# kishwarshafin/pepper

Hardware: AMD Instinct MI355X
Metric: inference windows/sec (whole node) (higher is better)
Workload: dtype f32 via f16 hi/lo split operands (3 MFMAs per product), f32 accumulate

## Files before the change

pepper_amd/build.py:

```python
import os
import shutil
import subprocess
import sys

CSRC = os.path.join(os.path.dirname(os.path.abspath(__file__)), "csrc")
LIB = os.path.join(CSRC, "libpepper_amd.so")
SOURCES = ["api.hip", "inflate.hip", "gemm.hip", "gemm_h2.hip", "rnn.hip", "rnn_h2.hip", "mlp_h2.hip", "head.hip", "encoder.hip", "encoder_polish.hip", "realign.hip"]
HEADERS = ["common.h", "kernels.h", "encoder_common.h", "reservoir.h", "candidates.h", "pack_rule.h", "dec_frag16.h", os.path.join("..", "..", "include", "pepper_amd.h"),
           os.path.join("..", "..", "include", "pepper_amd_encoder.h"),
           os.path.join("..", "..", "include", "pepper_amd_realign.h")]


def _hipcc():
    for cand in (os.environ.get("HIPCC"), shutil.which("hipcc"), "/opt/rocm/bin/hipcc"):
        if cand and os.path.exists(cand):
            return cand
    raise RuntimeError("hipcc not found (set HIPCC)")


IO_LIB = os.path.join(CSRC, "libpepper_amd_io.so")
HDF5_PREFIX = os.environ.get("PEPPER_AMD_HDF5_PREFIX", "/opt/conda")


def _have_libdeflate(inc, lib):
    if os.environ.get("PEPPER_AMD_LIBDEFLATE", "1") == "0":
        return False
    return os.path.exists(os.path.join(inc, "libdeflate.h")) and os.path.exists(os.path.join(lib, "libdeflate.so"))


def build_io(force=False, verbose=False):
    src = os.path.join(CSRC, "hdf5io.cpp")
    bam = os.path.join(CSRC, "bamio.cpp")
    bld = os.path.join(CSRC, "h5build.cpp")
    cnd = os.path.join(CSRC, "candidates.cpp")
    hdr = os.path.join(CSRC, "..", "..", "include", "pepper_amd_io.h")
    rsv = os.path.join(CSRC, "reservoir.h")
    pkr = os.path.join(CSRC, "pack_rule.h")
    have_src = all(os.path.exists(f) for f in (src, bam, bld, cnd, hdr, rsv, pkr))
    if os.path.exists(IO_LIB) and (not have_src or (not force and os.path.getmtime(IO_LIB) >= max(
            os.path.getmtime(src), os.path.getmtime(bam), os.path.getmtime(bld), os.path.getmtime(cnd), os.path.getmtime(hdr),
            os.path.getmtime(rsv), os.path.getmtime(pkr)))):
        return IO_LIB
    inc, lib = os.path.join(HDF5_PREFIX, "include"), os.path.join(HDF5_PREFIX, "lib")
    if not os.path.exists(os.path.join(inc, "hdf5.h")):
        raise RuntimeError(f"hdf5.h not found under {inc}: set PEPPER_AMD_HDF5_PREFIX")
    tmp = f"{IO_LIB}.{os.getpid()}.tmp"
    cmd = ["g++", "-O2", "-std=c++17", "-shared", "-fPIC", "-o", tmp, src, bam, bld, cnd, f"-I{inc}",
           os.path.join(lib, "libhdf5.so"), "-lz", "-lpthread", f"-Wl,-rpath,{lib}", "-Wl,--no-undefined"]
    if _have_libdeflate(inc, lib):
        cmd += ["-DPA_HAVE_LIBDEFLATE=1", os.path.join(lib, "libdeflate.so")]
    if verbose:
        print(" ".join(cmd), file=sys.stderr)
    try:
        subprocess.run(cmd, check=True)
        os.replace(tmp, IO_LIB)
    finally:
        if os.path.exists(tmp):
            os.remove(tmp)
    return IO_LIB


TOOLS = os.path.join(os.path.dirname(os.path.dirname(os.path.abspath(__file__))), "tools")
SYNTH_BAM = os.path.join(TOOLS, "synth_bam")


def build_tools(force=False):
    src = os.path.join(TOOLS, "synth_bam.cpp")
    if not os.path.exists(src):
        return SYNTH_BAM if os.path.exists(SYNTH_BAM) else None
    if not force and os.path.exists(SYNTH_BAM) and os.path.getmtime(SYNTH_BAM) >= os.path.getmtime(src):
        return SYNTH_BAM
    inc, lib = os.path.join(HDF5_PREFIX, "include"), os.path.join(HDF5_PREFIX, "lib")
    tmp = f"{SYNTH_BAM}.{os.getpid()}.tmp"
    cmd = ["g++", "-O2", "-std=c++17", "-o", tmp, src, "-lz", "-lpthread"]
    if _have_libdeflate(inc, lib):
        cmd += [f"-I{inc}", "-DPA_HAVE_LIBDEFLATE=1", os.path.join(lib, "libdeflate.so"), f"-Wl,-rpath,{lib}"]
    try:
        subprocess.run(cmd, check=True)
        os.replace(tmp, SYNTH_BAM)
    finally:
        if os.path.exists(tmp):
            os.remove(tmp)
    return SYNTH_BAM


OBJ_DIR = os.path.join(CSRC, "_obj")


def _flags():
    return ["--offload-arch=gfx950", "-O3", "-std=c++17", "-fPIC", "-Xarch_host", "-mf16c", "-Wno-unused-result"] + \
        os.environ.get("PEPPER_AMD_EXTRA_HIPCC_FLAGS", "").split()


def _same_flags():
    stamp = os.path.join(OBJ_DIR, "flags.txt")
    return not os.path.exists(stamp) or open(stamp).read() == " ".join(_flags())


def needs_build():
    if not os.path.exists(LIB):
        return True
    t = os.path.getmtime(LIB)
    return not _same_flags() or any(os.path.getmtime(os.path.join(CSRC, f)) > t for f in SOURCES + HEADERS)


def build(force=False, verbose=False):
    if not force and not needs_build():
        return LIB
    flags = _flags()
    os.makedirs(OBJ_DIR, exist_ok=True)
    stamp = os.path.join(OBJ_DIR, "flags.txt")
    same_flags = os.path.exists(stamp) and open(stamp).read() == " ".join(flags)
    newest_header = max(os.path.getmtime(os.path.join(CSRC, h)) for h in HEADERS)
    todo = []
    for src in SOURCES:
        obj = os.path.join(OBJ_DIR, src + ".o")
        if force or not same_flags or not os.path.exists(obj) or os.path.getmtime(obj) < max(
                newest_header, os.path.getmtime(os.path.join(CSRC, src))):
            todo.append((src, obj))

    def compile_one(item):
        src, obj = item
        cmd = [_hipcc()] + flags + ["-c", src, "-o", obj + f".{os.getpid()}.tmp"]
        if verbose:
            print(" ".join(cmd), file=sys.stderr)
        subprocess.run(cmd, cwd=CSRC, check=True)
        os.replace(obj + f".{os.getpid()}.tmp", obj)
    if todo:
        from concurrent.futures import ThreadPoolExecutor
        with ThreadPoolExecutor(max_workers=min(len(todo), os.cpu_count() or 4)) as pool:
            list(pool.map(compile_one, todo))
    with open(stamp, "w") as fh:
        fh.write(" ".join(flags))
    tmp = f"{LIB}.{os.getpid()}.tmp"
    cmd = [_hipcc(), "--offload-arch=gfx950", "-shared", "-fPIC", "-o", tmp] + [os.path.join(OBJ_DIR, s + ".o") for s in SOURCES]
    if verbose:
        print(" ".join(cmd), file=sys.stderr)
    try:
        subprocess.run(cmd, cwd=CSRC, check=True)
        os.replace(tmp, LIB)
    finally:
        if os.path.exists(tmp):
            os.remove(tmp)
    return LIB


if __name__ == "__main__":
    print(build(force=True, verbose=True))
    print(build_io(force=True, verbose=True))
    print(build_tools(force=True))
```

pepper_amd/csrc/rnn_h2.hip:

```cpp
#include <cstdlib>

#include "common.h"
#include "kernels.h"

namespace {

typedef _Float16 h8 __attribute__((ext_vector_type(8)));

constexpr int MT = 64;

PA_DEV f32x16 mfma_h(h8 a, h8 b, f32x16 c) { return __builtin_amdgcn_mfma_f32_32x32x16_f16(a, b, c, 0, 0, 0); }

PA_DEV void decode_block(int bid, int& dir, int& btile) {
    const int xcd = bid & 7, q = bid >> 3;
    dir = xcd >> 2;
    btile = q * 4 + (xcd & 3);
}



template <int MTILES>
PA_DEV void lstm_dec_h2_body(const float* __restrict__ bias, const uint32_t* __restrict__ Wp, uint32_t* __restrict__ Y, int ldy,
                             int B, int T, unsigned long long* __restrict__ dbg, const uint32_t* __restrict__ Xh, int ldxh);
template <int MTILES, bool BC>
PA_DEV void lstm_enc_h2_body(const int8_t* __restrict__ Xi, int F, const float* __restrict__ bias, const uint32_t* __restrict__ Wp,
                             uint32_t* __restrict__ Y, int ldy, int B, int T, unsigned long long* __restrict__ dbg);

template <int H, int KX, bool XG = false, int SAUX = 0, bool BC = false, int MTILES = 2>
__global__ __launch_bounds__(H / 32 * 64, 1) void lstm_rec_h2_kernel(const float* __restrict__ Xp, int ldx,
                                                                     const int8_t* __restrict__ Xi, int F,
                                                                     const float* __restrict__ bias,
                                                                     const uint32_t* __restrict__ Wp,
                                                                     uint32_t* __restrict__ Y, int ldy, int B, int T,
                                                                     unsigned long long* __restrict__ dbg,
                                                                     const uint32_t* __restrict__ Xh = nullptr, int ldxh = 0) {
    if constexpr (XG) {
        static_assert(H == 256 && KX == 512 && SAUX == 2 && !BC, "the fused decoder has one shape");
        lstm_dec_h2_body<MTILES>(bias, Wp, Y, ldy, B, T, dbg, Xh, ldxh);
        return;
    }
    if constexpr (!XG && KX == 32) {
        static_assert(H == 256 && SAUX == 2, "the fused int8 encoder has one shape");
        lstm_enc_h2_body<MTILES, BC>(Xi, F, bias, Wp, Y, ldy, B, T, dbg);
        return;
    }
    constexpr int KT = H + KX, KS = KT / 16, KSH = H / 16, NT = H / 32, NW = H / 32;
    constexpr int MTL = 32 * MTILES;
    static_assert(MTILES == 1 || MTILES == 2, "32 or 64 rows per workgroup");
    constexpr int ROWB = KT * 4 + 16;
    constexpr int ROWD = ROWB / 4;
    extern __shared__ __attribute__((aligned(16))) uint32_t lds[];
    static_assert(KS % 2 == 0, "the weight prefetch assumes an even number of k steps");
    static_assert((ROWB / 16) % 2 == 1, "row stride must be an odd number of 16-byte slots");

    int dir, btile;
    decode_block(blockIdx.x, dir, btile);
    const int b0 = btile * MTL;
    if (b0 >= B) return;

    const int tid = threadIdx.x, lane = tid & 63;
    const int u = __builtin_amdgcn_readfirstlane(tid >> 6);
    const int li = lane & 31, hf = lane >> 5;

    float* cs = reinterpret_cast<float*>(lds + MTL * ROWD) + u * (MTILES * 16 * 64) + lane;
    for (int idx = tid; idx < MTL * ROWD + NW * MTILES * 16 * 64; idx += blockDim.x) lds[idx] = 0u;

    f32x16 acc[MTILES][4];

    const size_t urow = (size_t)b0 * T;
    const __amdgpu_buffer_rsrc_t xrs = __builtin_amdgcn_make_buffer_rsrc(
        const_cast<float*>(KX ? bias + dir * 4 * H + 32 * u : Xp + (size_t)(b0 >> 5) * T * (ldx >> 5) * 1024), 0,
        0x7fffffff, 0x00020000);
    const __amdgpu_buffer_rsrc_t wrs = __builtin_amdgcn_make_buffer_rsrc(
        const_cast<uint32_t*>(Wp + ((size_t)dir * (4 * NT) + u) * KS * 512), 0, 0x7fffffff, 0x00020000);
    const unsigned xoff = KX ? li * 4u : lane * 16u;
    const unsigned woff = lane * 16u;

    auto seed_chunk = [&](int m, int qd, int t) {
        if (KX) return;
#pragma unroll
        for (int g = 0; g < 4; ++g) {
            {
                const unsigned ct = (unsigned)(dir * (4 * NT) + g * NT + u);
                const unsigned so = (((unsigned)(m * T + t) * (ldx >> 5) + ct) * 4u + qd) * 1024u;
                const f32x4 v = __builtin_bit_cast(f32x4, __builtin_amdgcn_raw_buffer_load_b128(xrs, xoff, so, 0));
                acc[m][g][4 * qd] = v.x;
                acc[m][g][4 * qd + 1] = v.y;
                acc[m][g][4 * qd + 2] = v.z;
                acc[m][g][4 * qd + 3] = v.w;
            }
        }
    };

    constexpr bool XI8 = KX > 0;
    constexpr int XN = XI8 ? (MTL * KX / 2) / (NW * 64) : 1;
    unsigned xv[XN];
    auto x_load = [&](int t) {
        if (XI8) {
#pragma unroll
            for (int k = 0; k < XN; ++k) {
                const int e = tid + k * (NW * 64);
                const int row = e / (KX / 2), f = (e % (KX / 2)) * 2;
                int brow = b0 + row;
                brow = brow < B ? brow : B - 1;
                const int8_t* src = Xi + ((size_t)brow * T + t) * F;
                const _Float16 one = BC ? (_Float16)1.0f : (_Float16)0.0f;
                const _Float16 h0 = f < F ? (_Float16)(float)src[f] : (f == F ? one : (_Float16)0.0f);
                const _Float16 h1 = f + 1 < F ? (_Float16)(float)src[f + 1] : (f + 1 == F ? one : (_Float16)0.0f);
                xv[k] = (unsigned)__builtin_bit_cast(unsigned short, h0) |
                        ((unsigned)__builtin_bit_cast(unsigned short, h1) << 16);
            }
        }
    };
    auto x_store = [&]() {
        if (XI8) {
#pragma unroll
            for (int k = 0; k < XN; ++k) {
                const int e = tid + k * (NW * 64);
                const int row = e / (KX / 2), f = (e % (KX / 2)) * 2;
                lds[row * ROWD + ((H + f) >> 3) * 8 + ((f & 7) >> 1)] = xv[k];
            }
        }
    };
    struct Frag { h8 b[4][2], a[MTILES][2]; };
    const uint32_t* arow = lds + li * ROWD + hf * 8;
    auto load_b = [&](int s, Frag& fr) {
#pragma unroll
        for (int g = 0; g < 4; ++g)
#pragma unroll
            for (int hl = 0; hl < 2; ++hl)
                fr.b[g][hl] = __builtin_bit_cast(h8, __builtin_amdgcn_raw_buffer_load_b128(
                                                         wrs, woff, (unsigned)((g * NT * KS + s) * 2 + hl) * 1024u, 0));
    };
    auto load_a = [&](int s, Frag& fr, int) {
#pragma unroll
        for (int m = 0; m < MTILES; ++m) {
            fr.a[m][0] = *reinterpret_cast<const h8*>(arow + m * 32 * ROWD + s * 16);
            fr.a[m][1] = *reinterpret_cast<const h8*>(arow + m * 32 * ROWD + s * 16 + 4);
        }
    };

    constexpr int CPR = H / 4;
    constexpr int YROWS = (NW * 64) / CPR;
    constexpr int YC = MTL / YROWS;
    const int yc_row = tid / CPR, yc_c = tid % CPR;
    const uint32_t* yc_src = lds + yc_row * ROWD + yc_c * 4;
    const __amdgpu_buffer_rsrc_t ycrs =
        __builtin_amdgcn_make_buffer_rsrc(Y + urow * ldy + dir * H, 0, 0x7fffffff, 0x00020000);
    const unsigned yc_off = ((unsigned)(yc_row * T) * ldy + yc_c * 4) * 4u;
    auto yc_read = [&](int j) { return *reinterpret_cast<const u32x4*>(yc_src + j * YROWS * ROWD); };
    auto yc_write = [&](int j, int tp, u32x4 v) {
        __builtin_amdgcn_raw_buffer_store_b128(v, ycrs, yc_off, ((unsigned)(j * YROWS * T + tp) * ldy) * 4u, SAUX);
    };

    const int hcol = 32 * u + li;
    unsigned short* hl_dst = reinterpret_cast<unsigned short*>(lds + 4 * hf * ROWD + (hcol >> 3) * 8 + ((hcol & 7) >> 1)) + (hcol & 1);
    const bool odd = li & 1;

    Frag ring[2];
    __syncthreads();
    {
        const int t0 = dir ? T - 1 : 0;
#pragma unroll
        for (int m = 0; m < MTILES; ++m)
#pragma unroll
            for (int qd = 0; qd < 4; ++qd) seed_chunk(m, qd, t0);
        x_load(t0);
        x_store();
        load_b(0, ring[0]);
    }
    __syncthreads();

    for (int step = 0; step < T; ++step) {
        const int t = dir ? T - 1 - step : step;
        const bool stamp = dbg != nullptr && blockIdx.x == 8 && lane == 0;
        if (stamp) dbg[(u * 80 + 2 * step) * 2] = __builtin_amdgcn_s_memtime();
        {
            load_a(0, ring[0], t);
            const int tp = step > 0 ? (dir ? t + 1 : t - 1) : t;
            u32x4 ycv = {0, 0, 0, 0};
#pragma unroll
            for (int s = 0; s < KS; ++s) {
                const int p = s & 1;
                if (s + 1 < KS) { load_b(s + 1, ring[p ^ 1]); load_a(s + 1, ring[p ^ 1], t); }
                else load_b(0, ring[p ^ 1]);
                if (s >= 1 && s <= YC) yc_write(s - 1, tp, ycv);
                if (s < YC) ycv = yc_read(s);
#pragma unroll
                for (int term = 0; term < 3; ++term) {
                    if (XI8 && s >= KSH && term == 0) continue;
                    const bool fresh = KX && s == 0 && term == 0;
#pragma unroll
                    for (int g = 0; g < 4; ++g)
#pragma unroll
                        for (int m = 0; m < MTILES; ++m)
                            acc[m][g] = mfma_h(ring[p].a[m][term == 0 ? 1 : 0], ring[p].b[g][term == 1 ? 1 : 0],
                                               fresh ? f32x16{} : acc[m][g]);
                }
                if (MTILES == 1 && s + 1 < KS) {
#pragma unroll
                    for (int q = 0; q < 8; ++q) {
                        __builtin_amdgcn_sched_group_barrier(0x008, 1, 0);
                        __builtin_amdgcn_sched_group_barrier(0x020, 1, 0);
                    }
#pragma unroll
                    for (int q = 0; q < 2; ++q) {
                        __builtin_amdgcn_sched_group_barrier(0x008, 1, 0);
                        __builtin_amdgcn_sched_group_barrier(0x100, 1, 0);
                    }
                    if (s <= YC) {
                        __builtin_amdgcn_sched_group_barrier(0x008, 1, 0);
                        __builtin_amdgcn_sched_group_barrier(0x040, 1, 0);
                        __builtin_amdgcn_sched_group_barrier(0x008, 1, 0);
                        __builtin_amdgcn_sched_group_barrier(0x100, 1, 0);
                    } else {
                        __builtin_amdgcn_sched_group_barrier(0x008, 2, 0);
                    }
                } else if (s + 1 < KS) {
#pragma unroll
                    for (int q = 0; q < 8; ++q) {
                        __builtin_amdgcn_sched_group_barrier(0x008, 2, 0);
                        __builtin_amdgcn_sched_group_barrier(0x020, 1, 0);
                    }
#pragma unroll
                    for (int q = 0; q < 4; ++q) {
                        __builtin_amdgcn_sched_group_barrier(0x008, 1, 0);
                        __builtin_amdgcn_sched_group_barrier(0x100, 1, 0);
                    }
                    if (s <= YC) {
                        __builtin_amdgcn_sched_group_barrier(0x008, 1, 0);
                        __builtin_amdgcn_sched_group_barrier(0x040, 1, 0);
                        __builtin_amdgcn_sched_group_barrier(0x008, 1, 0);
                        __builtin_amdgcn_sched_group_barrier(0x100, 1, 0);
                        __builtin_amdgcn_sched_group_barrier(0x008, 2, 0);
                    } else {
                        __builtin_amdgcn_sched_group_barrier(0x008, 4, 0);
                    }
                } else if (MTILES == 1) {
#pragma unroll
                    for (int q = 0; q < 8; ++q) {
                        __builtin_amdgcn_sched_group_barrier(0x008, 1, 0);
                        __builtin_amdgcn_sched_group_barrier(0x020, 1, 0);
                    }
                    __builtin_amdgcn_sched_group_barrier(0x008, 4, 0);
                } else {
#pragma unroll
                    for (int q = 0; q < 8; ++q) {
                        __builtin_amdgcn_sched_group_barrier(0x008, 2, 0);
                        __builtin_amdgcn_sched_group_barrier(0x020, 1, 0);
                    }
                    __builtin_amdgcn_sched_group_barrier(0x008, 8, 0);
                }
                __builtin_amdgcn_sched_barrier(0);
            }
        }
        float cb[4] = {0.0f, 0.0f, 0.0f, 0.0f};
        if (KX && !BC) {
#pragma unroll
            for (int g = 0; g < 4; ++g)
                cb[g] = __builtin_bit_cast(float, __builtin_amdgcn_raw_buffer_load_b32(xrs, xoff, (unsigned)(g * H) * 4u, 0));
        }
        if (stamp) dbg[(u * 80 + 2 * step) * 2 + 1] = __builtin_amdgcn_s_memtime();

        lds_barrier();
        if (stamp) dbg[(u * 80 + 2 * step + 1) * 2] = __builtin_amdgcn_s_memtime();

        const int tn = dir ? t - 1 : t + 1;
        if (step + 1 < T) x_load(tn);
#pragma unroll
        for (int m = 0; m < MTILES; ++m)
#pragma unroll
            for (int qd = 0; qd < 4; ++qd) {
#pragma unroll
                for (int e = 0; e < 4; e += 2) {
                    const int r = 4 * qd + e;
                    typedef float f32x2 __attribute__((ext_vector_type(2)));
                    const f32x2 one = {1.0f, 1.0f};
                    f32x2 ai = {acc[m][0][r], acc[m][0][r + 1]}, af = {acc[m][1][r], acc[m][1][r + 1]},
                          ag = {acc[m][2][r], acc[m][2][r + 1]}, ao = {acc[m][3][r], acc[m][3][r + 1]};
                    if (KX && !BC) { ai += cb[0]; af += cb[1]; ag += cb[2]; ao += cb[3]; }
                    auto ex2 = [](f32x2 v) { return f32x2{__builtin_amdgcn_exp2f(v.x), __builtin_amdgcn_exp2f(v.y)}; };
                    auto rcp = [](f32x2 v) { return f32x2{__builtin_amdgcn_rcpf(v.x), __builtin_amdgcn_rcpf(v.y)}; };
                    const f32x2 ig = rcp(one + ex2(ai));
                    const f32x2 fg = rcp(one + ex2(af));
                    const f32x2 gg = one - 2.0f * rcp(one + ex2(ag));
                    const f32x2 og = rcp(one + ex2(ao));
                    const f32x2 cold = {cs[(m * 16 + r) * 64], cs[(m * 16 + r + 1) * 64]};
                    const f32x2 cn = fg * cold + ig * gg;
                    cs[(m * 16 + r) * 64] = cn.x;
                    cs[(m * 16 + r + 1) * 64] = cn.y;
                    const f32x2 hv2 = og * (one - 2.0f * rcp(one + ex2(cn * 2.8853900817779268f)));
#pragma unroll
                    for (int k = 0; k < 2; ++k) {
                        const float hv = k ? hv2.y : hv2.x;
                        h2_store16(hl_dst + (32 * m + ((r + k) & 3) + 8 * ((r + k) >> 2)) * ROWD * 2, hv);
                    }
                }
                if (step + 1 < T) seed_chunk(m, qd, tn);
            }
        if (step + 1 < T) x_store();
        if (stamp) dbg[(u * 80 + 2 * step + 1) * 2 + 1] = __builtin_amdgcn_s_memtime();
        lds_barrier();
    }
    {
        const int tl = dir ? 0 : T - 1;
#pragma unroll
        for (int j = 0; j < YC; ++j) yc_write(j, tl, yc_read(j));
    }
}

template <bool FRESH_, bool Y_, bool Y2_, int XR_, int AN_>
struct DecStep {
    static constexpr bool FRESH = FRESH_, Y = Y_, Y2 = Y2_;
    static constexpr int XR = XR_, AN = AN_;
};

template <int MTILES>
PA_DEV void lstm_dec_h2_body(const float* __restrict__ bias, const uint32_t* __restrict__ Wp, uint32_t* __restrict__ Y, int ldy,
                             int B, int T, unsigned long long* __restrict__ dbg, const uint32_t* __restrict__ Xh, int ldxh) {
    constexpr int H = 256, KX = 512, KS = (H + KX) / 32, KSH = H / 32, NW = H / 32, SAUX = 2;
    constexpr int MTL = 32 * MTILES, RT = 2 * MTILES;
    static_assert(MTILES == 1 || MTILES == 2, "32 or 64 rows per workgroup");
    constexpr int ROWB = H * 4 + 16, ROWD = ROWB / 4;
    extern __shared__ __attribute__((aligned(16))) uint32_t lds[];
    static_assert((ROWB / 16) % 2 == 1, "row stride must be an odd number of 16-byte slots");

    int dir, btile;
    decode_block(blockIdx.x, dir, btile);
    const int b0 = btile * MTL;
    if (b0 >= B) return;

    const int tid = threadIdx.x, lane = tid & 63;
    const int u = __builtin_amdgcn_readfirstlane(tid >> 6);
    const int lr = lane & 15, lq = lane >> 4;

    float* cs = reinterpret_cast<float*>(lds + MTL * ROWD) + u * (MTILES * 16 * 64) + lane;
    for (int idx = tid; idx < MTL * ROWD + NW * MTILES * 16 * 64; idx += blockDim.x) lds[idx] = 0u;
    constexpr int XRD = 36, XSLOT = MTL * XRD;
    uint32_t* xring = lds + MTL * ROWD + NW * MTILES * 16 * 64;

    f32x4 acc[RT][4][2];

    const size_t urow = (size_t)b0 * T;
    const __amdgpu_buffer_rsrc_t brs =
        __builtin_amdgcn_make_buffer_rsrc(const_cast<float*>(bias + dir * 4 * H + 32 * u), 0, 0x7fffffff, 0x00020000);
    const __amdgpu_buffer_rsrc_t wrs = __builtin_amdgcn_make_buffer_rsrc(
        const_cast<uint32_t*>(Wp + ((size_t)dir * (4 * 16) + 2 * u) * KS * 512), 0, 0x7fffffff, 0x00020000);
    const unsigned woff = lane * 16u;

    const bool xg_stager = tid < MTL * 8;
    const __amdgpu_buffer_rsrc_t xgrs =
        __builtin_amdgcn_make_buffer_rsrc(const_cast<uint32_t*>(Xh + (size_t)b0 * T * ldxh), 0, 0x7fffffff, 0x00020000);
    const unsigned xg_off = ((unsigned)((tid >> 3) * T) * ldxh) * 4u + (tid & 7) * 16u;
    uint32_t* xst_dst = xring + (tid >> 3) * XRD + (tid & 7) * 4;
    u32x4 xstage = {0, 0, 0, 0};
    auto xg_load = [&](int j, int t) {
        if (MTILES == 2 || xg_stager)
            xstage = __builtin_amdgcn_raw_buffer_load_b128(xgrs, xg_off, ((unsigned)t * ldxh) * 4u + (unsigned)j * 128u, SAUX);
    };
    auto xg_store = [&](int slot) {
        if (MTILES == 2 || xg_stager) *reinterpret_cast<u32x4*>(xst_dst + slot * XSLOT) = xstage;
    };

    int once = 1;
    asm volatile("" : "+s"(once));
    h8 a[RT][2];
    h8 b[2][2][2][2];
    const uint32_t* arow = lds + lr * ROWD + lq * 8;
    const uint32_t* xrow = xring + lr * XRD + lq * 8;
    auto load_b = [&](int s, int gp, int idx) {
        const int c = idx >> 2, hl = (idx >> 1) & 1, g2 = idx & 1;
        b[gp][g2][c][hl] = __builtin_bit_cast(
            h8, __builtin_amdgcn_raw_buffer_load_b128(wrs, woff, (unsigned)((((2 * gp + g2) * 16 + c) * KS + s) * 2 + hl) * 1024u, 0));
    };
    auto load_a_h = [&](int s, int m, int hl) { a[m][hl] = *reinterpret_cast<const h8*>(arow + m * 16 * ROWD + s * 32 + hl * 4); };
    auto load_a_x = [&](int slot, int m, int hl) {
        a[m][hl] = *reinterpret_cast<const h8*>(xrow + slot * XSLOT + m * 16 * XRD + hl * 4);
    };

    constexpr int CPR = H / 4;
    constexpr int YROWS = (NW * 64) / CPR;
    constexpr int YC = MTL / YROWS;
    const int yc_row = tid / CPR, yc_c = tid % CPR;
    const uint32_t* yc_src = lds + yc_row * ROWD + yc_c * 4;
    const __amdgpu_buffer_rsrc_t ycrs =
        __builtin_amdgcn_make_buffer_rsrc(Y + urow * ldy + dir * H, 0, 0x7fffffff, 0x00020000);
    const unsigned yc_off = ((unsigned)(yc_row * T) * ldy + yc_c * 4) * 4u;
    auto yc_read = [&](int j) { return *reinterpret_cast<const u32x4*>(yc_src + j * YROWS * ROWD); };
    auto yc_write = [&](int j, int tp, u32x4 v) {
        __builtin_amdgcn_raw_buffer_store_b128(v, ycrs, yc_off, ((unsigned)(j * YROWS * T + tp) * ldy) * 4u, SAUX);
    };

    const int hcol = 32 * u + lr;
    unsigned short* hl_dst = reinterpret_cast<unsigned short*>(lds + 4 * lq * ROWD + (hcol >> 3) * 8 + ((hcol & 7) >> 1)) + (hcol & 1);

    __syncthreads();
#pragma unroll
    for (int i = 0; i < 8; ++i) load_b(0, 0, i);
    __syncthreads();

    for (int step = 0; step < T; ++step) {
        const int t = dir ? T - 1 - step : step;
        const bool stamp = dbg != nullptr && blockIdx.x == 8 && lane == 0;
        if (stamp) dbg[(u * 80 + 2 * step) * 2] = __builtin_amdgcn_s_memtime();
        {
            const int tp = step > 0 ? (dir ? t + 1 : t - 1) : t;
            u32x4 ycv = {0, 0, 0, 0}, ycv2 = {0, 0, 0, 0};
            constexpr int NM = RT * 12;
            auto kstep = [&](int s, auto cfg) {
                using C = decltype(cfg);
                const int sn = C::AN == 0 ? 0 : s + 1, slot = (s - KSH + 1) & 1;
#pragma unroll
                for (int gp = 0; gp < 2; ++gp) {
                    if (gp == 1 && C::XR == 2) lds_barrier();
#pragma unroll
                    for (int i = 0; i < NM; ++i) {
                        const int m = i / 12, c = (i % 12) / 6, term = (i % 6) >> 1, g2 = i & 1, g = 2 * gp + g2;
                        acc[m][g][c] = __builtin_amdgcn_mfma_f32_16x16x32_f16(a[m][term == 0 ? 1 : 0], b[gp][g2][c][term == 1 ? 1 : 0],
                                                                              C::FRESH && term == 0 ? f32x4{} : acc[m][g][c], 0, 0, 0);
                        if (MTILES == 2 ? (i < 24 && i % 3 == 1) : i < 8) load_b(gp == 0 ? s : sn, gp ^ 1, MTILES == 2 ? i / 3 : i);
                        if (gp == 1 && C::AN != 0 && (i % 12 == 9 || i % 12 == 11)) {
                            if (C::AN == 1) load_a_h(sn, m, i % 12 == 9 ? 1 : 0);
                            else load_a_x(slot, m, i % 12 == 9 ? 1 : 0);
                        }
                        if (C::Y && i == NM / 2 + 1) {
                            if (gp == 0) ycv = yc_read(s);
                            else yc_write(s, tp, ycv);
                        }
                        if (C::Y2 && i == NM / 2 + 4) {
                            if (gp == 0) ycv2 = yc_read(YC - 1);
                            else yc_write(YC - 1, tp, ycv2);
                        }
                        if (C::XR == 2 && gp == 0 && i == NM - 1) xg_store(slot);
                        if (C::XR != 0 && gp == 1 && i == (MTILES == 2 ? 2 : 10)) xg_load(s - 6 < KS - KSH ? s - 6 : KS - KSH - 1, t);
                        __builtin_amdgcn_sched_barrier(0);
                    }
                }
            };
            constexpr bool Y2 = YC > 7;
            constexpr int YL = YC < 6 ? YC : 6;
#pragma unroll
            for (int i = 0; i < 2 * RT; ++i) load_a_h(0, i >> 1, i & 1);
            __builtin_amdgcn_sched_barrier(0);
#pragma unroll 1
            for (int r = 0; r < once; ++r) kstep(0, DecStep<true, true, Y2, 0, 1>{});
#pragma unroll 1
            for (int s = 1; s < YL; ++s) kstep(s, DecStep<false, true, false, 0, 1>{});
#pragma unroll 1
            for (int s = YL; s < 6; ++s) kstep(s, DecStep<false, false, false, 0, 1>{});
#pragma unroll 1
            for (int r = 0; r < once; ++r) kstep(6, DecStep<false, (YC > 6), false, 1, 1>{});
#pragma unroll 1
            for (int s = 7; s < KS - 1; ++s) kstep(s, DecStep<false, false, false, 2, 2>{});
#pragma unroll 1
            for (int r = 0; r < once; ++r) kstep(KS - 1, DecStep<false, false, false, 0, 0>{});
        }
        float cb[4][2];
#pragma unroll
        for (int g = 0; g < 4; ++g)
#pragma unroll
            for (int c = 0; c < 2; ++c)
                cb[g][c] = __builtin_bit_cast(float, __builtin_amdgcn_raw_buffer_load_b32(brs, lr * 4u, (unsigned)(g * H + 16 * c) * 4u, 0));
        if (stamp) dbg[(u * 80 + 2 * step) * 2 + 1] = __builtin_amdgcn_s_memtime();

        lds_barrier();
        if (stamp) dbg[(u * 80 + 2 * step + 1) * 2] = __builtin_amdgcn_s_memtime();

#pragma unroll
        for (int m = 0; m < RT; ++m)
#pragma unroll
            for (int c = 0; c < 2; ++c)
#pragma unroll
                for (int e = 0; e < 4; e += 2) {
                    typedef float f32x2 __attribute__((ext_vector_type(2)));
                    const f32x2 one = {1.0f, 1.0f};
                    f32x2 ai = {acc[m][0][c][e], acc[m][0][c][e + 1]}, af = {acc[m][1][c][e], acc[m][1][c][e + 1]},
                          ag = {acc[m][2][c][e], acc[m][2][c][e + 1]}, ao = {acc[m][3][c][e], acc[m][3][c][e + 1]};
                    ai += cb[0][c]; af += cb[1][c]; ag += cb[2][c]; ao += cb[3][c];
                    auto ex2 = [](f32x2 v) { return f32x2{__builtin_amdgcn_exp2f(v.x), __builtin_amdgcn_exp2f(v.y)}; };
                    auto rcp = [](f32x2 v) { return f32x2{__builtin_amdgcn_rcpf(v.x), __builtin_amdgcn_rcpf(v.y)}; };
                    const f32x2 ig = rcp(one + ex2(ai));
                    const f32x2 fg = rcp(one + ex2(af));
                    const f32x2 gg = one - 2.0f * rcp(one + ex2(ag));
                    const f32x2 og = rcp(one + ex2(ao));
                    const int ci = (m * 8 + c * 4 + e) * 64;
                    const f32x2 cold = {cs[ci], cs[ci + 64]};
                    const f32x2 cn = fg * cold + ig * gg;
                    cs[ci] = cn.x;
                    cs[ci + 64] = cn.y;
                    const f32x2 hv2 = og * (one - 2.0f * rcp(one + ex2(cn * 2.8853900817779268f)));
#pragma unroll
                    for (int k = 0; k < 2; ++k) h2_store16(hl_dst + (16 * m + e + k) * ROWD * 2 + c * 32, k ? hv2.y : hv2.x);
                }
        if (stamp) dbg[(u * 80 + 2 * step + 1) * 2 + 1] = __builtin_amdgcn_s_memtime();
        lds_barrier();
    }
    {
        const int tl = dir ? 0 : T - 1;
#pragma unroll
        for (int j = 0; j < YC; ++j) yc_write(j, tl, yc_read(j));
    }
}

#ifndef PA_ENC_SKIP0
#define PA_ENC_SKIP0 1
#endif
template <bool FRESH_, bool Y_, bool X_, int AN_>
struct EncStep {
    static constexpr bool FRESH = FRESH_, Y = Y_, X = X_;
    static constexpr int AN = AN_;
};

template <int MTILES, bool BC>
PA_DEV void lstm_enc_h2_body(const int8_t* __restrict__ Xi, int F, const float* __restrict__ bias, const uint32_t* __restrict__ Wp,
                             uint32_t* __restrict__ Y, int ldy, int B, int T, unsigned long long* __restrict__ dbg) {
    constexpr int H = 256, KX = 32, KS = (H + KX) / 32, KSH = H / 32, NW = H / 32, SAUX = 2;
    constexpr int MTL = 32 * MTILES, RT = 2 * MTILES;
    static_assert(MTILES == 1 || MTILES == 2, "32 or 64 rows per workgroup");
    constexpr int ROWB = (H + KX) * 4 + 16, ROWD = ROWB / 4;
    extern __shared__ __attribute__((aligned(16))) uint32_t lds[];
    static_assert((ROWB / 16) % 2 == 1, "row stride must be an odd number of 16-byte slots");

    int dir, btile;
    decode_block(blockIdx.x, dir, btile);
    const int b0 = btile * MTL;
    if (b0 >= B) return;

    const int tid = threadIdx.x, lane = tid & 63;
    const int u = __builtin_amdgcn_readfirstlane(tid >> 6);
    const int lr = lane & 15, lq = lane >> 4;

    float* cs = reinterpret_cast<float*>(lds + MTL * ROWD) + u * (MTILES * 16 * 64) + lane;
    for (int idx = tid; idx < MTL * ROWD + NW * MTILES * 16 * 64; idx += blockDim.x) lds[idx] = 0u;

    f32x4 acc[RT][4][2];

    const size_t urow = (size_t)b0 * T;
    const __amdgpu_buffer_rsrc_t brs =
        __builtin_amdgcn_make_buffer_rsrc(const_cast<float*>(bias + dir * 4 * H + 32 * u), 0, 0x7fffffff, 0x00020000);
    const __amdgpu_buffer_rsrc_t wrs = __builtin_amdgcn_make_buffer_rsrc(
        const_cast<uint32_t*>(Wp + ((size_t)dir * (4 * 16) + 2 * u) * KS * 512), 0, 0x7fffffff, 0x00020000);
    const unsigned woff = lane * 16u;

    constexpr int XN = (MTL * KX / 2) / (NW * 64);
    unsigned xv[XN];
    auto x_load = [&](int t) {
#pragma unroll
        for (int k = 0; k < XN; ++k) {
            const int e = tid + k * (NW * 64);
            const int row = e / (KX / 2), f = (e % (KX / 2)) * 2;
            int brow = b0 + row;
            brow = brow < B ? brow : B - 1;
            const int8_t* src = Xi + ((size_t)brow * T + t) * F;
            const _Float16 one = BC ? (_Float16)1.0f : (_Float16)0.0f;
            const _Float16 h0 = f < F ? (_Float16)(float)src[f] : (f == F ? one : (_Float16)0.0f);
            const _Float16 h1 = f + 1 < F ? (_Float16)(float)src[f + 1] : (f + 1 == F ? one : (_Float16)0.0f);
            xv[k] = (unsigned)__builtin_bit_cast(unsigned short, h0) | ((unsigned)__builtin_bit_cast(unsigned short, h1) << 16);
        }
    };
    auto x_store = [&]() {
#pragma unroll
        for (int k = 0; k < XN; ++k) {
            const int e = tid + k * (NW * 64);
            const int row = e / (KX / 2), f = (e % (KX / 2)) * 2;
            lds[row * ROWD + ((H + f) >> 3) * 8 + ((f & 7) >> 1)] = xv[k];
        }
    };

    int once = 1;
    asm volatile("" : "+s"(once));
    h8 a[RT][2];
    h8 b[2][2][2][2];
    const uint32_t* arow = lds + lr * ROWD + lq * 8;
    auto load_b = [&](int s, int gp, int idx) {
        const int c = idx >> 2, hl = (idx >> 1) & 1, g2 = idx & 1;
        b[gp][g2][c][hl] = __builtin_bit_cast(
            h8, __builtin_amdgcn_raw_buffer_load_b128(wrs, woff, (unsigned)((((2 * gp + g2) * 16 + c) * KS + s) * 2 + hl) * 1024u, 0));
    };
    auto load_a = [&](int s, int m, int hl) { a[m][hl] = *reinterpret_cast<const h8*>(arow + m * 16 * ROWD + s * 32 + hl * 4); };

    constexpr int CPR = H / 4;
    constexpr int YROWS = (NW * 64) / CPR;
    constexpr int YC = MTL / YROWS;
    static_assert(YC <= KSH, "one y copy pass per h k step");
    const int yc_row = tid / CPR, yc_c = tid % CPR;
    const uint32_t* yc_src = lds + yc_row * ROWD + yc_c * 4;
    const __amdgpu_buffer_rsrc_t ycrs =
        __builtin_amdgcn_make_buffer_rsrc(Y + urow * ldy + dir * H, 0, 0x7fffffff, 0x00020000);
    const unsigned yc_off = ((unsigned)(yc_row * T) * ldy + yc_c * 4) * 4u;
    auto yc_read = [&](int j) { return *reinterpret_cast<const u32x4*>(yc_src + j * YROWS * ROWD); };
    auto yc_write = [&](int j, int tp, u32x4 v) {
        __builtin_amdgcn_raw_buffer_store_b128(v, ycrs, yc_off, ((unsigned)(j * YROWS * T + tp) * ldy) * 4u, SAUX);
    };

    const int hcol = 32 * u + lr;
    unsigned short* hl_dst = reinterpret_cast<unsigned short*>(lds + 4 * lq * ROWD + (hcol >> 3) * 8 + ((hcol & 7) >> 1)) + (hcol & 1);

    __syncthreads();
    {
        x_load(dir ? T - 1 : 0);
        x_store();
#pragma unroll
        for (int i = 0; i < 8; ++i) load_b(PA_ENC_SKIP0 ? KS - 1 : 0, 0, i);
    }
    __syncthreads();

    for (int step = 0; step < T; ++step) {
        const int t = dir ? T - 1 - step : step;
        const bool stamp = dbg != nullptr && blockIdx.x == 8 && lane == 0;
        if (stamp) dbg[(u * 80 + 2 * step) * 2] = __builtin_amdgcn_s_memtime();
        {
            const int tp = step > 0 ? (dir ? t + 1 : t - 1) : t;
            u32x4 ycv = {0, 0, 0, 0};
            auto kstep = [&](int s, auto cfg) {
                using C = decltype(cfg);
                constexpr int PT = C::X ? 4 : 6;
                constexpr int NM = RT * 2 * PT;
                const int sn = C::X ? 0 : s + 1;
#pragma unroll
                for (int gp = 0; gp < 2; ++gp) {
#pragma unroll
                    for (int i = 0; i < NM; ++i) {
                        const int m = i / (2 * PT), c = (i % (2 * PT)) / PT, term = ((i % PT) >> 1) + (C::X ? 1 : 0), g2 = i & 1,
                                  g = 2 * gp + g2;
                        acc[m][g][c] = __builtin_amdgcn_mfma_f32_16x16x32_f16(a[m][term == 0 ? 1 : 0], b[gp][g2][c][term == 1 ? 1 : 0],
                                                                              C::FRESH && i % PT < 2 ? f32x4{} : acc[m][g][c], 0, 0, 0);
                        if (C::X) {
                            if (MTILES == 2 ? (i < 16 && (i & 1)) : i < 8) load_b(gp == 0 ? s : sn, gp ^ 1, MTILES == 2 ? i >> 1 : i);
                        } else {
                            if (MTILES == 2 ? (i < 24 && i % 3 == 1) : i < 8) load_b(gp == 0 ? s : sn, gp ^ 1, MTILES == 2 ? i / 3 : i);
                        }
                        if (!C::X && gp == 1 && C::AN == 1 && i % 12 == 9) load_a(sn, m, 1);
                        if (!C::X && gp == 1 && C::AN != 0 && i % 12 == 11) load_a(sn, m, 0);
                        if (C::Y && i == NM / 2 + 1) {
                            if (gp == 0) ycv = yc_read(s);
                            else yc_write(s, tp, ycv);
                        }
                        __builtin_amdgcn_sched_barrier(0);
                    }
                }
            };
            const int hrun = PA_ENC_SKIP0 && step == 0 ? 0 : once;
#pragma unroll
            for (int i = 0; i < 2 * RT; ++i) load_a(0, i >> 1, i & 1);
            __builtin_amdgcn_sched_barrier(0);
#pragma unroll 1
            for (int r = 0; r < hrun; ++r) kstep(0, EncStep<true, true, false, 1>{});
#pragma unroll 1
            for (int s = 1; s < (YC < KSH - 1 ? YC : KSH - 1) * hrun; ++s) kstep(s, EncStep<false, true, false, 1>{});
            if constexpr (YC < KSH - 1) {
#pragma unroll 1
                for (int s = YC; s < (KSH - 1) * hrun; ++s) kstep(s, EncStep<false, false, false, 1>{});
            }
#pragma unroll 1
            for (int r = 0; r < hrun; ++r) kstep(KSH - 1, EncStep<false, (YC >= KSH), false, 2>{});
#pragma unroll 1
            for (int r = 0; r < hrun; ++r) kstep(KS - 1, EncStep<false, false, true, 0>{});
            if (PA_ENC_SKIP0) {
#pragma unroll 1
                for (int r = hrun; r < once; ++r) {
#pragma unroll
                    for (int m = 0; m < RT; ++m) load_a(KSH, m, 0);
                    __builtin_amdgcn_sched_barrier(0);
                    kstep(KS - 1, EncStep<true, false, true, 0>{});
                }
            }
        }
        float cb[4][2] = {};
        if (!BC) {
#pragma unroll
            for (int g = 0; g < 4; ++g)
#pragma unroll
                for (int c = 0; c < 2; ++c)
                    cb[g][c] = __builtin_bit_cast(float, __builtin_amdgcn_raw_buffer_load_b32(brs, lr * 4u, (unsigned)(g * H + 16 * c) * 4u, 0));
        }
        if (stamp) dbg[(u * 80 + 2 * step) * 2 + 1] = __builtin_amdgcn_s_memtime();

        lds_barrier();
        if (stamp) dbg[(u * 80 + 2 * step + 1) * 2] = __builtin_amdgcn_s_memtime();

        const int tn = dir ? t - 1 : t + 1;
        if (step + 1 < T) x_load(tn);
#pragma unroll
        for (int m = 0; m < RT; ++m)
#pragma unroll
            for (int c = 0; c < 2; ++c)
#pragma unroll
                for (int e = 0; e < 4; e += 2) {
                    typedef float f32x2 __attribute__((ext_vector_type(2)));
                    const f32x2 one = {1.0f, 1.0f};
                    f32x2 ai = {acc[m][0][c][e], acc[m][0][c][e + 1]}, af = {acc[m][1][c][e], acc[m][1][c][e + 1]},
                          ag = {acc[m][2][c][e], acc[m][2][c][e + 1]}, ao = {acc[m][3][c][e], acc[m][3][c][e + 1]};
                    if (!BC) { ai += cb[0][c]; af += cb[1][c]; ag += cb[2][c]; ao += cb[3][c]; }
                    auto ex2 = [](f32x2 v) { return f32x2{__builtin_amdgcn_exp2f(v.x), __builtin_amdgcn_exp2f(v.y)}; };
                    auto rcp = [](f32x2 v) { return f32x2{__builtin_amdgcn_rcpf(v.x), __builtin_amdgcn_rcpf(v.y)}; };
                    const f32x2 ig = rcp(one + ex2(ai));
                    const f32x2 fg = rcp(one + ex2(af));
                    const f32x2 gg = one - 2.0f * rcp(one + ex2(ag));
                    const f32x2 og = rcp(one + ex2(ao));
                    const int ci = (m * 8 + c * 4 + e) * 64;
                    const f32x2 cold = {cs[ci], cs[ci + 64]};
                    const f32x2 cn = fg * cold + ig * gg;
                    cs[ci] = cn.x;
                    cs[ci + 64] = cn.y;
                    const f32x2 hv2 = og * (one - 2.0f * rcp(one + ex2(cn * 2.8853900817779268f)));
#pragma unroll
                    for (int k = 0; k < 2; ++k) h2_store16(hl_dst + (16 * m + e + k) * ROWD * 2 + c * 32, k ? hv2.y : hv2.x);
                }
        if (step + 1 < T) x_store();
        if (stamp) dbg[(u * 80 + 2 * step + 1) * 2 + 1] = __builtin_amdgcn_s_memtime();
        lds_barrier();
    }
    {
        const int tl = dir ? 0 : T - 1;
#pragma unroll
        for (int j = 0; j < YC; ++j) yc_write(j, tl, yc_read(j));
    }
}

constexpr int US_AUX_SC1 = 16;

template <int H, int NTW>
__global__ __launch_bounds__(256, 1) void lstm_rec_h2_split_kernel(const float* __restrict__ Xp, int ldx,
                                                                   const uint32_t* __restrict__ Wp, uint32_t* __restrict__ Y,
                                                                   int ldy, int B, int T, uint32_t* __restrict__ exch,
                                                                   unsigned* __restrict__ counters, int* __restrict__ failed,
                                                                   int tiles4, int sabotage) {
    static_assert(H == 256 && (NTW == 1 || NTW == 2), "eight members of 32 units or four of 64");
    constexpr int KS = H / 16, NT = H / 32, K = NT / NTW;
    constexpr int ROWB = H * 4 + 16, ROWD = ROWB / 4;
    extern __shared__ __attribute__((aligned(16))) uint32_t lds[];
    float* gbuf = reinterpret_cast<float*>(lds + 32 * ROWD);
    uint32_t* flag = lds + 32 * ROWD + 4 * NTW * 16 * 64;

    const int xcd = blockIdx.x & 7, q = blockIdx.x >> 3;
    const int dir = xcd >> 2, member = q % K, btile = (q / K) * 4 + (xcd & 3);
    const int b0 = btile * 32;
    if (b0 >= B) return;
    const int group = dir * tiles4 + btile;

    const int tid = threadIdx.x, lane = tid & 63;
    const int w = __builtin_amdgcn_readfirstlane(tid >> 6);
    const int li = lane & 31, hf = lane >> 5;
    for (int idx = tid; idx < 32 * ROWD; idx += 256) lds[idx] = 0u;
    if (tid == 0) *flag = 0u;

    h8 bw[NTW][KS][2];
    {
        const __amdgpu_buffer_rsrc_t wrs = __builtin_amdgcn_make_buffer_rsrc(
            const_cast<uint32_t*>(Wp + (size_t)dir * (4 * NT) * KS * 512), 0, 0x7fffffff, 0x00020000);
#pragma unroll
        for (int j = 0; j < NTW; ++j)
#pragma unroll
            for (int s = 0; s < KS; ++s)
#pragma unroll
                for (int hl = 0; hl < 2; ++hl)
                    bw[j][s][hl] = __builtin_bit_cast(h8, __builtin_amdgcn_raw_buffer_load_b128(
                                                              wrs, lane * 16u,
                                                              (unsigned)(((w * NT + member * NTW + j) * KS + s) * 2 + hl) * 1024u, 0));
    }
    const __amdgpu_buffer_rsrc_t xrs = __builtin_amdgcn_make_buffer_rsrc(
        const_cast<float*>(Xp + (size_t)btile * T * (ldx >> 5) * 1024), 0, 0x7fffffff, 0x00020000);
    const unsigned ct0 = (unsigned)(dir * (4 * NT) + w * NT + member * NTW);
    f32x16 acc[NTW];
    auto seed = [&](int t) {
#pragma unroll
        for (int j = 0; j < NTW; ++j)
#pragma unroll
            for (int qd = 0; qd < 4; ++qd) {
                const unsigned so = (((unsigned)t * (ldx >> 5) + ct0 + j) * 4u + qd) * 1024u;
                const f32x4 v = __builtin_bit_cast(f32x4, __builtin_amdgcn_raw_buffer_load_b128(xrs, lane * 16u, so, 0));
                acc[j][4 * qd] = v.x;
                acc[j][4 * qd + 1] = v.y;
                acc[j][4 * qd + 2] = v.z;
                acc[j][4 * qd + 3] = v.w;
            }
    };

    const uint32_t* arow = lds + li * ROWD + hf * 8;
    const int hcol = 32 * member * NTW + li;
    unsigned short* hl_dst = reinterpret_cast<unsigned short*>(lds + 4 * hf * ROWD + (hcol >> 3) * 8 + ((hcol & 7) >> 1)) + (hcol & 1);
    const int xrow = tid >> 3, xc = tid & 7;
    const __amdgpu_buffer_rsrc_t ers = __builtin_amdgcn_make_buffer_rsrc(
        exch + (size_t)group * 2 * 32 * H, 0, 0x7fffffff, 0x00020000);
    const __amdgpu_buffer_rsrc_t yrs = __builtin_amdgcn_make_buffer_rsrc(
        Y + (size_t)b0 * T * ldy + dir * H, 0, 0x7fffffff, 0x00020000);
    unsigned* cnt = counters + group * 32;

    float c[NTW][4];
#pragma unroll
    for (int j = 0; j < NTW; ++j)
#pragma unroll
        for (int e = 0; e < 4; ++e) c[j][e] = 0.0f;
    seed(dir ? T - 1 : 0);
    __syncthreads();

    for (int step = 0; step < T; ++step) {
        const int t = dir ? T - 1 - step : step;
        {
            h8 a0 = *reinterpret_cast<const h8*>(arow), a1 = *reinterpret_cast<const h8*>(arow + 4);
#pragma unroll
            for (int s = 0; s < KS; ++s) {
                h8 n0 = a0, n1 = a1;
                if (s + 1 < KS) {
                    n0 = *reinterpret_cast<const h8*>(arow + (s + 1) * 16);
                    n1 = *reinterpret_cast<const h8*>(arow + (s + 1) * 16 + 4);
                }
#pragma unroll
                for (int j = 0; j < NTW; ++j) acc[j] = mfma_h(a1, bw[j][s][0], acc[j]);
#pragma unroll
                for (int j = 0; j < NTW; ++j) acc[j] = mfma_h(a0, bw[j][s][1], acc[j]);
#pragma unroll
                for (int j = 0; j < NTW; ++j) acc[j] = mfma_h(a0, bw[j][s][0], acc[j]);
                a0 = n0;
                a1 = n1;
            }
        }
#pragma unroll
        for (int j = 0; j < NTW; ++j)
#pragma unroll
            for (int r = 0; r < 16; ++r) {
                const float sg = __builtin_amdgcn_rcpf(1.0f + __builtin_amdgcn_exp2f(acc[j][r]));
                gbuf[((w * NTW + j) * 16 + r) * 64 + lane] = w == 2 ? 1.0f - 2.0f * sg : sg;
            }
        if (step + 1 < T) seed(dir ? t - 1 : t + 1);
        lds_barrier();
#pragma unroll
        for (int j = 0; j < NTW; ++j)
#pragma unroll
            for (int e = 0; e < 4; ++e) {
                const int r = 4 * w + e;
                const float ig = gbuf[((0 * NTW + j) * 16 + r) * 64 + lane], fg = gbuf[((1 * NTW + j) * 16 + r) * 64 + lane];
                const float gg = gbuf[((2 * NTW + j) * 16 + r) * 64 + lane], og = gbuf[((3 * NTW + j) * 16 + r) * 64 + lane];
                const float cn = fg * c[j][e] + ig * gg;
                c[j][e] = cn;
                const float hv = og * (1.0f - 2.0f * __builtin_amdgcn_rcpf(1.0f + __builtin_amdgcn_exp2f(cn * 2.8853900817779268f)));
                h2_store16(hl_dst + j * 64 + (e + 8 * w) * ROWD * 2, hv);
            }
        lds_barrier();
        const unsigned pbase = (unsigned)(step & 1) * (32u * H * 4u);
#pragma unroll
        for (int j = 0; j < NTW; ++j) {
            const int chunk = (member * NTW + j) * 8 + xc;
            const u32x4 mine = *reinterpret_cast<const u32x4*>(lds + xrow * ROWD + chunk * 4);
            __builtin_amdgcn_raw_buffer_store_b128(mine, yrs, ((unsigned)(xrow * T) * ldy + chunk * 4) * 4u, ((unsigned)t * ldy) * 4u, 0);
            if (step + 1 < T)
                __builtin_amdgcn_raw_buffer_store_b128(mine, ers, (unsigned)(xrow * H + chunk * 4) * 4u, pbase, US_AUX_SC1);
        }
        if (step + 1 == T) break;
        __builtin_amdgcn_s_waitcnt(0);
        __builtin_amdgcn_s_barrier();
        if (tid == 0) {
            if (!(sabotage && group == 0 && member == K - 1))
                __hip_atomic_fetch_add(cnt, 1u, __ATOMIC_RELAXED, __HIP_MEMORY_SCOPE_AGENT);
            const unsigned want = (unsigned)K * (unsigned)(step + 1);
            const int bound = step == 0 ? (1 << 13) : (1 << 11);
            int spins = 0;
            while (__hip_atomic_load(cnt, __ATOMIC_RELAXED, __HIP_MEMORY_SCOPE_AGENT) < want) {
// ... 870 lines not shown
```

Baseline: 2.732 million.

## Fold LSTM gate math into fewer transcendentals and skip zero-state decoder step

Moves the LSTM cell nonlinearity into a shared header and adds a form that merges the input and candidate gates, and the output gate with the tanh of the cell, into single reciprocals, with clamped exponent arguments. The aim is to cut exp/rcp instructions in the serial recurrent step. The decoder also gains a step-zero path that skips the recurrent h-matmul k-steps, since the initial hidden state is zero, and loads the x operand earlier. The new gate form changes rounding slightly, and the step-zero path adds control-flow complexity to the k-step schedule.

After: 2.731 million (median of 2 runs). No clear change (-0.0%).

```diff
diff --git a/pepper_amd/build.py b/pepper_amd/build.py
--- a/pepper_amd/build.py
+++ b/pepper_amd/build.py
@@ -6,7 +6,7 @@
 CSRC = os.path.join(os.path.dirname(os.path.abspath(__file__)), "csrc")
 LIB = os.path.join(CSRC, "libpepper_amd.so")
 SOURCES = ["api.hip", "inflate.hip", "gemm.hip", "gemm_h2.hip", "rnn.hip", "rnn_h2.hip", "mlp_h2.hip", "head.hip", "encoder.hip", "encoder_polish.hip", "realign.hip"]
-HEADERS = ["common.h", "kernels.h", "encoder_common.h", "reservoir.h", "candidates.h", "pack_rule.h", "dec_frag16.h", os.path.join("..", "..", "include", "pepper_amd.h"),
+HEADERS = ["common.h", "kernels.h", "encoder_common.h", "reservoir.h", "candidates.h", "pack_rule.h", "dec_frag16.h", "lstm_gate.h", os.path.join("..", "..", "include", "pepper_amd.h"),
            os.path.join("..", "..", "include", "pepper_amd_encoder.h"),
            os.path.join("..", "..", "include", "pepper_amd_realign.h")]
 
diff --git a/pepper_amd/csrc/lstm_gate.h b/pepper_amd/csrc/lstm_gate.h
--- /dev/null
+++ b/pepper_amd/csrc/lstm_gate.h
@@ -0,0 +1,64 @@
+#pragma once
+#include <math.h>
+
+#ifndef PA_LSTM_GATE_FORM
+#define PA_LSTM_GATE_FORM 8
+#endif
+#if PA_LSTM_GATE_FORM != 10 && PA_LSTM_GATE_FORM != 8
+#error "PA_LSTM_GATE_FORM is 10 or 8"
+#endif
+
+namespace pa_gate {
+
+#if defined(__HIPCC__)
+#define PA_GATE_FN __host__ __device__ __forceinline__
+#else
+#define PA_GATE_FN inline
+#endif
+#if defined(__clang__)
+typedef float f32x2 __attribute__((ext_vector_type(2)));
+#else
+struct f32x2 {
+    float x, y;
+};
+inline f32x2 operator+(f32x2 a, f32x2 b) { return f32x2{a.x + b.x, a.y + b.y}; }
+inline f32x2 operator-(f32x2 a, f32x2 b) { return f32x2{a.x - b.x, a.y - b.y}; }
+inline f32x2 operator*(f32x2 a, f32x2 b) { return f32x2{a.x * b.x, a.y * b.y}; }
+#endif
+#if defined(__HIP_DEVICE_COMPILE__)
+PA_GATE_FN f32x2 ex2(f32x2 v) { return f32x2{__builtin_amdgcn_exp2f(v.x), __builtin_amdgcn_exp2f(v.y)}; }
+PA_GATE_FN f32x2 rcp(f32x2 v) { return f32x2{__builtin_amdgcn_rcpf(v.x), __builtin_amdgcn_rcpf(v.y)}; }
+PA_GATE_FN f32x2 at_most(f32x2 v, float hi) { return f32x2{__builtin_fminf(v.x, hi), __builtin_fminf(v.y, hi)}; }
+#else
+PA_GATE_FN f32x2 ex2(f32x2 v) { return f32x2{exp2f(v.x), exp2f(v.y)}; }
+PA_GATE_FN f32x2 rcp(f32x2 v) { return f32x2{1.0f / v.x, 1.0f / v.y}; }
+PA_GATE_FN f32x2 at_most(f32x2 v, float hi) { return f32x2{v.x < hi ? v.x : hi, v.y < hi ? v.y : hi}; }
+#endif
+
+PA_GATE_FN f32x2 both(float v) { return f32x2{v, v}; }
+PA_GATE_FN f32x2 fma2(f32x2 a, f32x2 b, f32x2 c) { return f32x2{__builtin_fmaf(a.x, b.x, c.x), __builtin_fmaf(a.y, b.y, c.y)}; }
+
+constexpr float TWO_LOG2E = 2.8853900817779268f;
+constexpr float ARG_MAX = 40.0f;
+
+template <int FORM>
+PA_GATE_FN f32x2 lstm_gate(f32x2 ai, f32x2 af, f32x2 ag, f32x2 ao, f32x2& c) {
+    static_assert(FORM == 10 || FORM == 8, "forms: 10 (reference), 8");
+    const f32x2 one = both(1.0f);
+    if (FORM == 10) {
+        const f32x2 ig = rcp(one + ex2(ai));
+        const f32x2 fg = rcp(one + ex2(af));
+        const f32x2 gg = one - both(2.0f) * rcp(one + ex2(ag));
+        const f32x2 og = rcp(one + ex2(ao));
+        c = fg * c + ig * gg;
+        return og * (one - both(2.0f) * rcp(one + ex2(c * both(TWO_LOG2E))));
+    } else {
+        const f32x2 eg = ex2(at_most(ag, ARG_MAX)), pg = one + eg;
+        const f32x2 fg = rcp(one + ex2(af));
+        c = fma2(fg, c, (eg - one) * rcp(fma2(ex2(ai), pg, pg)));
+        const f32x2 ec = ex2(at_most(c * both(TWO_LOG2E), ARG_MAX)), pc = one + ec;
+        return (ec - one) * rcp(fma2(ex2(ao), pc, pc));
+    }
+}
+
+}
diff --git a/pepper_amd/csrc/rnn_h2.hip b/pepper_amd/csrc/rnn_h2.hip
--- a/pepper_amd/csrc/rnn_h2.hip
+++ b/pepper_amd/csrc/rnn_h2.hip
@@ -2,6 +2,7 @@
 
 #include "common.h"
 #include "kernels.h"
+#include "lstm_gate.h"
 
 namespace {
 
@@ -274,22 +275,14 @@
 #pragma unroll
                 for (int e = 0; e < 4; e += 2) {
                     const int r = 4 * qd + e;
-                    typedef float f32x2 __attribute__((ext_vector_type(2)));
-                    const f32x2 one = {1.0f, 1.0f};
+                    using pa_gate::f32x2;
                     f32x2 ai = {acc[m][0][r], acc[m][0][r + 1]}, af = {acc[m][1][r], acc[m][1][r + 1]},
                           ag = {acc[m][2][r], acc[m][2][r + 1]}, ao = {acc[m][3][r], acc[m][3][r + 1]};
                     if (KX && !BC) { ai += cb[0]; af += cb[1]; ag += cb[2]; ao += cb[3]; }
-                    auto ex2 = [](f32x2 v) { return f32x2{__builtin_amdgcn_exp2f(v.x), __builtin_amdgcn_exp2f(v.y)}; };
-                    auto rcp = [](f32x2 v) { return f32x2{__builtin_amdgcn_rcpf(v.x), __builtin_amdgcn_rcpf(v.y)}; };
-                    const f32x2 ig = rcp(one + ex2(ai));
-                    const f32x2 fg = rcp(one + ex2(af));
-                    const f32x2 gg = one - 2.0f * rcp(one + ex2(ag));
-                    const f32x2 og = rcp(one + ex2(ao));
-                    const f32x2 cold = {cs[(m * 16 + r) * 64], cs[(m * 16 + r + 1) * 64]};
-                    const f32x2 cn = fg * cold + ig * gg;
+                    f32x2 cn = {cs[(m * 16 + r) * 64], cs[(m * 16 + r + 1) * 64]};
+                    const f32x2 hv2 = pa_gate::lstm_gate<PA_LSTM_GATE_FORM>(ai, af, ag, ao, cn);
                     cs[(m * 16 + r) * 64] = cn.x;
                     cs[(m * 16 + r + 1) * 64] = cn.y;
-                    const f32x2 hv2 = og * (one - 2.0f * rcp(one + ex2(cn * 2.8853900817779268f)));
 #pragma unroll
                     for (int k = 0; k < 2; ++k) {
                         const float hv = k ? hv2.y : hv2.x;
@@ -309,6 +302,9 @@
     }
 }
 
+#ifndef PA_DEC_SKIP0
+#define PA_DEC_SKIP0 1
+#endif
 template <bool FRESH_, bool Y_, bool Y2_, int XR_, int AN_>
 struct DecStep {
     static constexpr bool FRESH = FRESH_, Y = Y_, Y2 = Y2_;
@@ -396,7 +392,8 @@
 
     __syncthreads();
 #pragma unroll
-    for (int i = 0; i < 8; ++i) load_b(0, 0, i);
+    for (int i = 0; i < 8; ++i) load_b(PA_DEC_SKIP0 ? KSH : 0, 0, i);
+    if (PA_DEC_SKIP0) xg_load(0, dir ? T - 1 : 0);
     __syncthreads();
 
     for (int step = 0; step < T; ++step) {
@@ -442,16 +439,29 @@
 #pragma unroll
             for (int i = 0; i < 2 * RT; ++i) load_a_h(0, i >> 1, i & 1);
             __builtin_amdgcn_sched_barrier(0);
+            const int hrun = PA_DEC_SKIP0 && step == 0 ? 0 : once;
 #pragma unroll 1
-            for (int r = 0; r < once; ++r) kstep(0, DecStep<true, true, Y2, 0, 1>{});
+            for (int r = 0; r < hrun; ++r) kstep(0, DecStep<true, true, Y2, 0, 1>{});
 #pragma unroll 1
-            for (int s = 1; s < YL; ++s) kstep(s, DecStep<false, true, false, 0, 1>{});
+            for (int s = 1; s < YL * hrun; ++s) kstep(s, DecStep<false, true, false, 0, 1>{});
 #pragma unroll 1
-            for (int s = YL; s < 6; ++s) kstep(s, DecStep<false, false, false, 0, 1>{});
+            for (int s = YL; s < 6 * hrun; ++s) kstep(s, DecStep<false, false, false, 0, 1>{});
 #pragma unroll 1
-            for (int r = 0; r < once; ++r) kstep(6, DecStep<false, (YC > 6), false, 1, 1>{});
+            for (int r = 0; r < hrun; ++r) kstep(6, DecStep<false, (YC > 6), false, 1, 1>{});
+            if (PA_DEC_SKIP0) {
 #pragma unroll 1
-            for (int s = 7; s < KS - 1; ++s) kstep(s, DecStep<false, false, false, 2, 2>{});
+                for (int r = hrun; r < once; ++r) {
+                    xg_store(0);
+                    lds_barrier();
+                    xg_load(1, t);
+#pragma unroll
+                    for (int i = 0; i < 2 * RT; ++i) load_a_x(0, i >> 1, i & 1);
+                    __builtin_amdgcn_sched_barrier(0);
+                    kstep(KSH, DecStep<true, false, false, 2, 2>{});
+                }
+            }
+#pragma unroll 1
+            for (int s = hrun ? KSH - 1 : KSH + 1; s < KS - 1; ++s) kstep(s, DecStep<false, false, false, 2, 2>{});
 #pragma unroll 1
             for (int r = 0; r < once; ++r) kstep(KS - 1, DecStep<false, false, false, 0, 0>{});
         }
@@ -472,23 +482,15 @@
             for (int c = 0; c < 2; ++c)
 #pragma unroll
                 for (int e = 0; e < 4; e += 2) {
-                    typedef float f32x2 __attribute__((ext_vector_type(2)));
-                    const f32x2 one = {1.0f, 1.0f};
+                    using pa_gate::f32x2;
                     f32x2 ai = {acc[m][0][c][e], acc[m][0][c][e + 1]}, af = {acc[m][1][c][e], acc[m][1][c][e + 1]},
                           ag = {acc[m][2][c][e], acc[m][2][c][e + 1]}, ao = {acc[m][3][c][e], acc[m][3][c][e + 1]};
                     ai += cb[0][c]; af += cb[1][c]; ag += cb[2][c]; ao += cb[3][c];
-                    auto ex2 = [](f32x2 v) { return f32x2{__builtin_amdgcn_exp2f(v.x), __builtin_amdgcn_exp2f(v.y)}; };
-                    auto rcp = [](f32x2 v) { return f32x2{__builtin_amdgcn_rcpf(v.x), __builtin_amdgcn_rcpf(v.y)}; };
-                    const f32x2 ig = rcp(one + ex2(ai));
-                    const f32x2 fg = rcp(one + ex2(af));
-                    const f32x2 gg = one - 2.0f * rcp(one + ex2(ag));
-                    const f32x2 og = rcp(one + ex2(ao));
                     const int ci = (m * 8 + c * 4 + e) * 64;
-                    const f32x2 cold = {cs[ci], cs[ci + 64]};
-                    const f32x2 cn = fg * cold + ig * gg;
+                    f32x2 cn = {cs[ci], cs[ci + 64]};
+                    const f32x2 hv2 = pa_gate::lstm_gate<PA_LSTM_GATE_FORM>(ai, af, ag, ao, cn);
                     cs[ci] = cn.x;
                     cs[ci + 64] = cn.y;
-                    const f32x2 hv2 = og * (one - 2.0f * rcp(one + ex2(cn * 2.8853900817779268f)));
 #pragma unroll
                     for (int k = 0; k < 2; ++k) h2_store16(hl_dst + (16 * m + e + k) * ROWD * 2 + c * 32, k ? hv2.y : hv2.x);
                 }
@@ -687,23 +689,15 @@
             for (int c = 0; c < 2; ++c)
 #pragma unroll
                 for (int e = 0; e < 4; e += 2) {
-                    typedef float f32x2 __attribute__((ext_vector_type(2)));
-                    const f32x2 one = {1.0f, 1.0f};
+                    using pa_gate::f32x2;
                     f32x2 ai = {acc[m][0][c][e], acc[m][0][c][e + 1]}, af = {acc[m][1][c][e], acc[m][1][c][e + 1]},
                           ag = {acc[m][2][c][e], acc[m][2][c][e + 1]}, ao = {acc[m][3][c][e], acc[m][3][c][e + 1]};
                     if (!BC) { ai += cb[0][c]; af += cb[1][c]; ag += cb[2][c]; ao += cb[3][c]; }
-                    auto ex2 = [](f32x2 v) { return f32x2{__builtin_amdgcn_exp2f(v.x), __builtin_amdgcn_exp2f(v.y)}; };
-                    auto rcp = [](f32x2 v) { return f32x2{__builtin_amdgcn_rcpf(v.x), __builtin_amdgcn_rcpf(v.y)}; };
-                    const f32x2 ig = rcp(one + ex2(ai));
-                    const f32x2 fg = rcp(one + ex2(af));
-                    const f32x2 gg = one - 2.0f * rcp(one + ex2(ag));
-                    const f32x2 og = rcp(one + ex2(ao));
                     const int ci = (m * 8 + c * 4 + e) * 64;
-                    const f32x2 cold = {cs[ci], cs[ci + 64]};
-                    const f32x2 cn = fg * cold + ig * gg;
+                    f32x2 cn = {cs[ci], cs[ci + 64]};
+                    const f32x2 hv2 = pa_gate::lstm_gate<PA_LSTM_GATE_FORM>(ai, af, ag, ao, cn);
                     cs[ci] = cn.x;
                     cs[ci + 64] = cn.y;
-                    const f32x2 hv2 = og * (one - 2.0f * rcp(one + ex2(cn * 2.8853900817779268f)));
 #pragma unroll
                     for (int k = 0; k < 2; ++k) h2_store16(hl_dst + (16 * m + e + k) * ROWD * 2 + c * 32, k ? hv2.y : hv2.x);
                 }
```
